# ChrisHird/ZLIB

Measured on AMD Instinct MI355X. Metric: GiB/s raw input compressed (deflate level 6), higher is better.
Workload: dtype u8

## Files before the change

### zlib_amd/csrc/zgpu_lz_parse.h

```cpp
#pragma once
#include "zgpu_common.h"

namespace zgpu {

#ifndef ZGPU_P2WIN
#define ZGPU_P2WIN 8192
#endif
constexpr uint32_t kP2Win = ZGPU_P2WIN, kP2Blk = kP2Win / 64;
constexpr uint32_t kP2Words = kChunkMax / 32, kP2Batch = 8, kP2Pair = 4, kP2Over = 8;
constexpr uint32_t kNone = 0xffffffffu;

struct ParseCtx {
    const uint2 *rec;
    uint32_t n, base, good, lazy, strategy;
    int slide_at;
    __device__ bool slid(uint32_t p) const { return (int)p >= slide_at; }
    __device__ uint32_t take(uint32_t p, uint32_t prev_len, uint2 r, uint32_t &dist) const
    {
        const uint32_t pick = (prev_len >= good && strategy != kRle) ? r.y : r.x;
        const uint32_t d = (pick >> 9) & 32767u;
        const bool nil = ((r.y >> 24) & 1u) && slid(p);
        const uint32_t len = nil ? 0u : (pick & 511u);
        const bool weak = len <= 5 && (strategy == kFiltered || (len == kMinMatch && d > kTooFar));
        const bool ok = prev_len < lazy && len > prev_len && !weak;
// ... 28 lines not shown
}

#if defined(ZGPU_P2_TIME) && !defined(ZGPU_PARSE_HEADER_ONLY)
__device__ unsigned long long p2_time[8];
extern "C" __attribute__((visibility("default"))) void zgpu_debug_p2_time(unsigned long long *out, int reset)
{
    unsigned long long z[8] = {};
    hipMemcpyFromSymbol(out, HIP_SYMBOL(p2_time), sizeof z);
    if (reset) hipMemcpyToSymbol(HIP_SYMBOL(p2_time), z, sizeof z);
}
#define P2_T(i) do { if (tid == 0) { const unsigned long long t_ = wall_clock64(); t_acc[i] += t_ - t_prev; t_prev = t_; } } while (0)
#define P2_T0() unsigned long long t_prev = wall_clock64(), t_acc[8] = {0, 0, 0, 0, 0, 0, 0, 0}
#define P2_TEND() do { if (tid == 0) for (int i_ = 0; i_ < 8; i_++) atomicAdd(&p2_time[i_], t_acc[i_]); } while (0)
#else
#define P2_T(i) do { } while (0)
#define P2_T0() do { } while (0)
#define P2_TEND() do { } while (0)
#endif

template <bool FUSED> __device__ inline uint32_t p2_ld(const uint32_t *p) { return FUSED ? __hip_atomic_load(p, __ATOMIC_RELAXED, __HIP_MEMORY_SCOPE_AGENT) : *p; }
constexpr uint32_t kP2OffJ = 0, kP2OffHAS = kP2Win * 2, kP2OffMARK = kP2OffHAS + kP2Words * 4, kP2OffCOV = kP2OffMARK + kP2Words * 4, kP2OffMAT = kP2OffCOV + kP2Words * 4,
                   kP2OffWbase = kP2OffMAT + kP2Words * 4, kP2OffVIS = kP2OffWbase + (kP2Words + 4) * 4, kP2OffEXITS = kP2OffVIS + kP2Win / 32 * 4, kP2OffWtot = kP2OffEXITS + 256,
                   kP2OffEntry = kP2OffWtot + 64, kP2LdsBytes = kP2OffEntry + 16;

}
```

### zlib_amd/csrc/zgpu_lz_parse.hip

```cpp
#include "zgpu_lz_parse.h"
#include "zgpu_engine.h"

namespace zgpu {

template <bool LITE, bool TILE>
__global__ void __launch_bounds__(1024, 8) parse2_kernel(ChunkGeom g, LevelCfg cfg, const uint2 *__restrict__ recs, const uint32_t *__restrict__ gmv_all,
                                                         const uint32_t *__restrict__ gsv_all, uint32_t *__restrict__ tokens, ChunkMeta *meta, TileGeom tg)
{
    constexpr uint32_t kP2Threads = 1024;
    constexpr bool FUSED = false;
    __shared__ __attribute__((aligned(16))) uint16_t J[kP2Win];
    __shared__ uint32_t HAS[kP2Words], MARK[kP2Words], COV[kP2Words], MAT[kP2Words];
    __shared__ uint32_t wbase[kP2Words + 1];
    __shared__ uint32_t VIS[kP2Win / 32], EXITS[64];
    __shared__ uint32_t wave_tot[kP2Threads / 64];
    __shared__ uint32_t sh_entry, sh_exit;
    const uint32_t c = blockIdx.x;
#include "zgpu_lz_parse_body.inc"
}

void launch_parse2(const ChunkGeom &g, LevelCfg cfg, const uint2 *recs, uint32_t *tokens, ChunkMeta *meta, hipStream_t st)
{
    hipLaunchKernelGGL((parse2_kernel<false, false>), dim3(g.nchunks), dim3(1024), 0, st, g, cfg, recs, nullptr, nullptr, tokens, meta, TileGeom{});
}

void launch_parse_tile(const ChunkGeom &g, LevelCfg cfg, const uint32_t *gm, const uint32_t *gs, uint32_t *tokens, ChunkMeta *meta, const TileGeom &tg, hipStream_t st)
{
    hipLaunchKernelGGL((parse2_kernel<true, true>), dim3(g.nchunks), dim3(1024), 0, st, g, cfg, nullptr, gm, gs, tokens, meta, tg);
}

}
```

### zlib_amd/csrc/zgpu_lz_parse_body.inc

```
{
    constexpr uint32_t kP2Own = kP2Win / kP2Threads;
    static_assert(kP2Own % kP2Batch == 0 && kP2Threads >= kP2Win / 32 && kP2Threads / 64 <= 16, "workgroup size");
    const uint32_t tid = threadIdx.x, lane = tid & 63, wave = tid >> 6;
    uint64_t lo; uint32_t n;
    chunk_span(g, c, lo, n);
    ParseCtx cx;
    cx.rec = LITE ? nullptr : recs + (size_t)c * kChunkMax;
    const uint32_t *gmv = LITE ? gmv_all + (size_t)c * kChunkMax : nullptr, *gsv = LITE ? gsv_all + (size_t)c * kP2Words : nullptr;
    cx.n = n; cx.base = chunk_base(g, c); cx.good = cfg.good; cx.lazy = cfg.lazy; cx.strategy = cfg.strategy;
    {
        const int room = (int)(2 * kWSize - cx.base), b0 = (int)n < room ? (int)n : room;
        const int a = b0 - (int)kMinLookahead + 1, b = (int)(kWSize + kMaxDist) - (int)cx.base;
        cx.slide_at = a > b ? a : b;
    }
    uint32_t *tok = tokens + (size_t)c * kChunkMax;
    const uint8_t *src = g.in + lo;
    const uint32_t nwords = (n + 31) >> 5;
    uint32_t t_h1 = n, t_e = 0;
    if (TILE) {
        uint64_t wb_; uint32_t nl_, h0_, ne_;
        tile_span(g, tg, c, wb_, nl_, h0_, t_h1, ne_);
        t_e = h0_ + tg.entry[g.chunk0 + c];
    }

    P2_T0();
    for (uint32_t i = tid; i < kP2Words; i += kP2Threads) { MARK[i] = 0; COV[i] = 0; MAT[i] = 0; if (LITE) HAS[i] = p2_ld<FUSED>(gsv + i); }
    if (!LITE) for (uint32_t p0 = 0; p0 < kChunkMax; p0 += kP2Threads * kP2Batch) {
        uint2 rv[kP2Batch];
#pragma unroll
        for (uint32_t u = 0; u < kP2Batch; u++) { const uint32_t p = p0 + u * kP2Threads + tid; rv[u] = p < n ? cx.rec[p] : make_uint2(0, 0); }
#pragma unroll
        for (uint32_t u = 0; u < kP2Batch; u++) {
            const uint32_t pw = p0 + u * kP2Threads, p = pw + tid;
            uint32_t d;
            const bool h = p < n && cx.take(p, kMinMatch - 1, rv[u], d) >= kMinMatch;
            const unsigned long long b = __builtin_amdgcn_ballot_w64(h);
            if (lane == 0) { HAS[(pw >> 5) + 2 * wave] = (uint32_t)b; HAS[(pw >> 5) + 2 * wave + 1] = (uint32_t)(b >> 32); }
        }
    }
    __syncthreads();
    if (tid == 0) {
        uint32_t x0 = (!TILE || t_e < t_h1) ? next_bit(HAS, t_e, nwords) : kNone;
        if (TILE && x0 != kNone && x0 >= t_h1) x0 = kNone;
        sh_entry = x0;
        if (TILE) sh_exit = t_e;
    }
    __syncthreads();
    P2_T(0);

    const uint32_t *TOK = COV;
    auto index_of = [&](uint32_t p) { return wbase[p >> 5] + (uint32_t)__builtin_popcount(TOK[p >> 5] & ~(~0u << (p & 31u))); };
    uint32_t tokbase = 0;
    uint32_t def_m = kNone, def_tok = 0;

    const uint32_t w_first = TILE ? t_e / kP2Win * kP2Win : 0u, w_lim = TILE ? (t_h1 + kTileSlack < n ? t_h1 + kTileSlack : n) : n;
    for (uint32_t w0 = w_first; w0 < w_lim; w0 += kP2Win) {
        const uint32_t wend = w0 + kP2Win;
        const uint32_t entry = sh_entry;
        uint32_t gm[kP2Own];
        uint32_t onp = 0;
#pragma unroll
        for (uint32_t i = 0; i < kP2Own; i++) gm[i] = 0;
        if (entry != kNone && entry < wend) {
            if (LITE) {
                uint32_t gv[kP2Own];
#pragma unroll
                for (uint32_t i = 0; i < kP2Own; i++) {
                    const uint32_t p = w0 + i * kP2Threads + tid;
#if defined(ZGPU_P2_EXP) && ZGPU_P2_EXP == 1
                    gv[i] = 0x00018001u;
#else
                    gv[i] = p < n ? p2_ld<FUSED>(gmv + p) : 0;
#endif
                }
#pragma unroll
                for (uint32_t i = 0; i < kP2Own; i++) {
                    const uint32_t p = w0 + i * kP2Threads + tid;
                    if (!(p < n && ((HAS[p >> 5] >> (p & 31u)) & 1u))) gv[i] = 0;
                }
#pragma unroll
                for (uint32_t i = 0; i < kP2Own; i++) {
                    const uint32_t xw = i * kP2Threads + tid, p = w0 + xw;
                    uint32_t succ = 0xffffu;
                    gm[i] = gv[i];
                    if (gv[i]) {
                        const uint32_t t = next_bit(HAS, p + (gv[i] >> 24) + ((gv[i] >> 15) & 511u), nwords);
                        if (t < wend) succ = t - w0;
// ... 125 lines not shown
                        if (x2 != kNone && x2 < be2) {
                            const uint32_t cw = (x2 - w0) >> 5;
                            if (lane < kP2Blk / 32) {
                                const uint32_t wd = blk * (kP2Blk / 32) + lane;
                                uint32_t v = VIS[wd];
                                if (wd < cw) v = 0; else if (wd == cw) v &= ~0u << (x2 & 31u);
                                if (v) atomicOr(&MARK[(w0 >> 5) + wd], v);
                            }
                            met_blk = blk;
                            x2 = EXITS[blk];
                        }
                        cur = (uint32_t)__builtin_amdgcn_readfirstlane(x2);
                        last = (uint32_t)__builtin_amdgcn_readfirstlane(last);
                        met_blk = (uint32_t)__builtin_amdgcn_readfirstlane(met_blk);
                    }
                    if (met_blk != kNone) {
                        uint32_t hi = 0;
                        for (uint32_t j = 0; j < kP2Blk / 32; j++) { const uint32_t v = VIS[met_blk * (kP2Blk / 32) + j]; if (v) hi = ((met_blk * (kP2Blk / 32) + j) << 5) + 32u - (uint32_t)__builtin_clz(v); }
                        last = w0 + hi - 1;
                    }
                }
                if (lane == 0) {
                    uint32_t m, L, D;
                    if (LITE) { const uint32_t gv = p2_ld<FUSED>(gmv + last); m = last + (gv >> 24); L = (gv >> 15) & 511u; D = gv & 32767u; }
                    else cx.game(last, cx.rec[last], cx.rec[last + 1], m, L, D);
                    sh_entry = next_bit(HAS, m + L, nwords);
                    if (TILE) sh_exit = m + L;
                }
            }
            __syncthreads();
            P2_T(2);
#pragma unroll
            for (uint32_t i = 0; i < kP2Own; i++) {
                const uint32_t p = w0 + i * kP2Threads + tid;
                const bool on_path = gm[i] != 0 && ((MARK[p >> 5] >> (p & 31u)) & 1u);
                onp |= on_path ? 1u << i : 0u;
                if (on_path) {
                    const uint32_t m = p + (gm[i] >> 24), L = (gm[i] >> 15) & 511u;
                    atomicOr(&MAT[m >> 5], 1u << (m & 31u));
                    const uint32_t a = m + 1, z = m + L;
                    for (uint32_t wd = a >> 5; wd <= (z - 1) >> 5; wd++) {
                        const uint32_t lo_b = wd == (a >> 5) ? (a & 31u) : 0u, hi_b = wd == ((z - 1) >> 5) ? ((z - 1) & 31u) : 31u;
                        atomicOr(&COV[wd], (~0u << lo_b) & (~0u >> (31u - hi_b)));
                    }
                }
            }
        }
        __syncthreads();
        P2_T(3);
        {
            const uint32_t wd = (w0 >> 5) + tid;
            uint32_t tw = 0;
            if (tid < kP2Win / 32 && wd < nwords) {
                tw = ~COV[wd];
                if (wd == nwords - 1 && (n & 31u)) tw &= ~0u >> (32u - (n & 31u));
                if (TILE) {
                    const uint32_t xl = wend > t_h1 ? (sh_exit > t_h1 ? sh_exit : t_h1) : wend, p0 = wd << 5;
// ... 10 lines not shown
            uint32_t b = tokbase + x - cnt, tot = 0;
            for (uint32_t w = 0; w < kP2Win / 32 / 64; w++) { const uint32_t t = wave_tot[w]; tot += t; if (w < wave) b += t; }
            if (tid < kP2Win / 32) { wbase[wd] = b; COV[wd] = tw; }
            tokbase += tot;
            __syncthreads();
        }
        P2_T(4);
        if (def_m != kNone) { tok[index_of(def_m)] = def_tok; def_m = kNone; }
#pragma unroll
        for (uint32_t ib = 0; ib < kP2Own; ib += kP2Batch) {
            uint32_t lit[kP2Batch];
            bool li[kP2Batch];
#pragma unroll
            for (uint32_t u = 0; u < kP2Batch; u++) {
                const uint32_t p = w0 + (ib + u) * kP2Threads + tid, bit = 1u << (p & 31u);
                li[u] = p < n && (TOK[p >> 5] & bit) && !(MAT[p >> 5] & bit);
                lit[u] = 0;
                if (p < n) lit[u] = src[p];
            }
#pragma unroll
            for (uint32_t u = 0; u < kP2Batch; u++) {
                const uint32_t p = w0 + (ib + u) * kP2Threads + tid;
                if (li[u]) tok[index_of(p)] = tok_lit(lit[u]);
                const uint32_t gv = ((onp >> (ib + u)) & 1u) ? gm[ib + u] : 0u;
                if (gv) {
                    const uint32_t m = p + (gv >> 24), t = tok_match(gv & 32767u, ((gv >> 15) & 511u) - kMinMatch);
                    if (m < wend) tok[index_of(m)] = t; else { def_m = m; def_tok = t; }
                }
            }
        }
        P2_T(5);
    }
    const uint32_t ntok = tokbase, nw_done = ((n + kP2Win - 1) / kP2Win) * (kP2Win / 32);
    __syncthreads();

    if (TILE) { if (tid == 0) { meta[c].ntok = ntok; meta[c].in_bytes = (sh_exit > t_h1 ? sh_exit : t_h1) - t_e; } }
    else if (tid == 0) {
        uint32_t nostore = 0, nblk = 0, block_start = 0;
        for (uint32_t b = 0;; b++) {
            const uint32_t e = (b + 1) * kBlockTokens - 1;
            if (e >= ntok) break;
            uint32_t lo_w = 0, hi_w = nw_done;
            while (hi_w - lo_w > 1) { const uint32_t mid = (lo_w + hi_w) >> 1; if (wbase[mid] <= e) lo_w = mid; else hi_w = mid; }
            uint32_t v = TOK[lo_w];
            for (uint32_t s2 = e - wbase[lo_w]; s2; s2--) v &= v - 1;
            const uint32_t pe = (lo_w << 5) + (uint32_t)__builtin_ctz(v);
            const bool is_mat = (MAT[pe >> 5] >> (pe & 31u)) & 1u;
            if (!is_mat && pe == n - 1) { nostore |= kFullFinalBlock; break; }
            uint32_t ns = pe + 1;
// ... 11 lines not shown
```

### zlib_amd/csrc/zgpu_lz_sorted.hip

```cpp
#include "zgpu_common.h"
#include "zgpu_engine.h"
#define ZGPU_PARSE_HEADER_ONLY
#include "zgpu_lz_parse.h"
#include <cstdlib>
#include "../../include/zamd_gpu.h"

#include <atomic>
static std::atomic<int> g_inject_sort_fault{0};
extern "C" __attribute__((visibility("default"))) void zgpu_debug_inject_sort_fault(void) { g_inject_sort_fault.store(1); }

namespace zgpu {

__device__ inline uint32_t lds_off(const void *p) { return (uint32_t)(uintptr_t)(const __attribute__((address_space(3))) void *)p; }
__device__ inline void lds_st32(uint32_t a, uint32_t v) { asm volatile("ds_write_b32 %0, %1" ::"v"(a), "v"(v) : "memory"); }
__device__ inline void lds_st16(uint32_t a, uint32_t v) { asm volatile("ds_write_b16 %0, %1" ::"v"(a), "v"(v) : "memory"); }
__device__ inline void lds_max32(uint32_t a, uint32_t v) { asm volatile("ds_max_u32 %0, %1" ::"v"(a), "v"(v) : "memory"); }
__device__ inline uint32_t lds_ld32(uint32_t a) { uint32_t v; asm volatile("ds_read_b32 %0, %1\n\ts_waitcnt lgkmcnt(0)" : "=v"(v) : "v"(a) : "memory"); return v; }
__device__ inline uint32_t lds_ld16(uint32_t a) { uint32_t v; asm volatile("ds_read_u16 %0, %1\n\ts_waitcnt lgkmcnt(0)" : "=v"(v) : "v"(a) : "memory"); return v; }

__device__ inline void lds_st8(uint32_t a, uint32_t v) { asm volatile("ds_write_b8 %0, %1" ::"v"(a), "v"(v) : "memory"); }
__device__ inline uint32_t lds_ld8(uint32_t a) { uint32_t v; asm volatile("ds_read_u8 %0, %1\n\ts_waitcnt lgkmcnt(0)" : "=v"(v) : "v"(a) : "memory"); return v; }

constexpr uint32_t kSuperS = 1024;

constexpr uint32_t kHeadWords = kChunkMax / 32;
constexpr uint32_t kHeadStride = kHeadWords + kChunkMax / 64 / 2;
constexpr uint32_t kGPad = 32, kGStride = kChunkMax + 2 * kGPad;

struct SortedWs {
    static constexpr size_t kHeaderBytes = 256, kSBytes = kSStride * 2, kRkBytes = kChunkMax * 2, kHeadBytes = kHeadStride * 4, kRecBytes = kChunkMax * 8, kIrBytes = kChunkMax * 4;
    static constexpr size_t kSlack = 1024;
    static_assert(kChunkMax * 4 + kChunkMax / 8 <= kRecBytes && kGStride <= kRecBytes, "gm + gs, and G, lie in the records' memory");
    static size_t bytes(size_t nchunks) { return kHeaderBytes + nchunks * (kSBytes + kRkBytes + kHeadBytes + kRecBytes + kIrBytes) + kSlack; }

    size_t nch;
    uint32_t *fault; uint16_t *S, *rk; uint32_t *heads; uint2 *recs; uint32_t *ir;
    SortedWs(void *workspace, size_t nchunks) : nch(nchunks)
    {
        uint8_t *p = static_cast<uint8_t *>(workspace);
        auto take = [&p](size_t n) { uint8_t *at = p; p += n; return at; };
        fault = reinterpret_cast<uint32_t *>(take(kHeaderBytes));
        S = reinterpret_cast<uint16_t *>(take((nch * kSBytes + 255) & ~(size_t)255));
        rk = reinterpret_cast<uint16_t *>(take(nch * kRkBytes));
        heads = reinterpret_cast<uint32_t *>(take(nch * kHeadBytes));
        recs = reinterpret_cast<uint2 *>(take(nch * kRecBytes));
        ir = reinterpret_cast<uint32_t *>(take(nch * kIrBytes));
    }
    uint32_t *gm() const { return reinterpret_cast<uint32_t *>(recs); }
    uint32_t *gs() const { return gm() + nch * kChunkMax; }
    uint8_t *G() const { return reinterpret_cast<uint8_t *>(recs); }
};

size_t lz_sorted_workspace_bytes(uint32_t batch) { return SortedWs::bytes(batch); }
uint32_t *lz_sorted_fault_word(void *workspace) { return SortedWs(workspace, 0).fault; }

__device__ inline uint32_t heads_below(unsigned long long x, uint32_t tid, uint32_t *wave_scratch)
{
    const uint32_t lane = tid & 63, wave = tid >> 6;
    const uint32_t v = x ? 64u * tid + 64u - (uint32_t)__builtin_clzll(x) : 0;
    uint32_t inc = v;
#pragma unroll
    for (int d = 1; d < 64; d <<= 1) { const uint32_t y = __shfl_up(inc, d); if ((int)lane >= d && y > inc) inc = y; }
    if (lane == 63) wave_scratch[wave] = inc;
    __syncthreads();
    uint32_t ex = __shfl_up(inc, 1);
    if (lane == 0) ex = 0;
    for (uint32_t w = 0; w < wave; w++) { const uint32_t y = wave_scratch[w]; if (y > ex) ex = y; }
    const uint32_t dist = 64u * tid - (ex - 1);
    return ex && dist < 65535u ? dist : 65535u;
}

__global__ void __launch_bounds__(1024) heads_below_kernel(uint32_t *__restrict__ heads_all)
// ... 531 lines not shown
            }
            if (p + base == kWSize + kMaxDist && avail != 0 && (uint32_t)sp[-1] + base == kWSize) flags = 1;
            rec[p] = make_uint2(full | ((uint32_t)d8[p] << 24), snap | (flags << 24));
        }
        blk = blk_nx;
    }
}

#ifndef ZGPU_WTRIG
#define ZGPU_WTRIG 48
#endif
#ifndef ZGPU_WBLK
#define ZGPU_WBLK 64
#endif
#ifndef ZGPU_WNEU_SHIFT
#define ZGPU_WNEU_SHIFT 0
#endif
#ifndef ZGPU_WFOLD_AT
#define ZGPU_WFOLD_AT 64
#endif
constexpr uint32_t kWFoldAt = ZGPU_WFOLD_AT;
constexpr uint32_t kWThreads = 512, kWWaves = kWThreads / 64, kWBlk = ZGPU_WBLK, kWTrig = ZGPU_WTRIG, kWNeuShift = ZGPU_WNEU_SHIFT;
constexpr uint32_t kWNeuBytes = (kChunkMax >> kWNeuShift) / 8;
constexpr uint32_t kWLds = kM3DataLds + 16 + kWNeuBytes + kWWaves * kM3WaveLds;
static_assert(2 * kWLds <= 160 * 1024, "two walker workgroups per CU");
enum : uint32_t { W_NEED = 0, W_LIMBO = 1, W_READY = 2, W_SEARCH = 3, W_DONE = 4 };
#ifdef ZGPU_WALK_STATS
__device__ unsigned long long walk_stats[8];
extern "C" __attribute__((visibility("default"))) void zgpu_debug_walk_stats(unsigned long long *out, int reset)
{
    unsigned long long z[8] = {};
    hipMemcpyFromSymbol(out, HIP_SYMBOL(walk_stats), sizeof z);
    if (reset) hipMemcpyToSymbol(HIP_SYMBOL(walk_stats), z, sizeof z);
}
#define W_STAT(i, v) do { const unsigned long long v_ = (unsigned long long)(v); if (lane == 0) atomicAdd(&walk_stats[i], v_); } while (0)
#else
#define W_STAT(i, v) do { } while (0)
#endif
#ifdef ZGPU_WALK_TIME
__device__ unsigned long long walk_time[8];
extern "C" __attribute__((visibility("default"))) void zgpu_debug_walk_time(unsigned long long *out, int reset)
{
    unsigned long long z[8] = {};
    hipMemcpyFromSymbol(out, HIP_SYMBOL(walk_time), sizeof z);
    if (reset) hipMemcpyToSymbol(HIP_SYMBOL(walk_time), z, sizeof z);
}
#define W_T0() unsigned long long wt_prev = __builtin_readcyclecounter(), wt_fold = 0, wt_lds = 0, wt_take = 0, wt_acc[8] = {0, 0, 0, 0, 0, 0, 0, 0}
#define W_T(i) do { const unsigned long long t_ = __builtin_readcyclecounter(); wt_acc[i] += t_ - wt_prev - ((i) == 1 ? wt_fold + wt_lds + wt_take : 0); \
                    if ((i) == 1) { wt_acc[2] += wt_fold; wt_acc[3] += wt_lds; wt_acc[7] += wt_take; } wt_fold = wt_lds = wt_take = 0; wt_prev = t_; } while (0)
#define W_TF(stmt) do { const unsigned long long f0_ = __builtin_readcyclecounter(); stmt; wt_fold += __builtin_readcyclecounter() - f0_; } while (0)
#define W_TL(stmt) do { const unsigned long long f0_ = __builtin_readcyclecounter(); stmt; wt_lds += __builtin_readcyclecounter() - f0_; } while (0)
#define W_TK(stmt) do { const unsigned long long f0_ = __builtin_readcyclecounter(); asm volatile("s_waitcnt vmcnt(0)" ::: "memory"); stmt; wt_take += __builtin_readcyclecounter() - f0_; } while (0)
#define W_TEND() do { if (lane == 0) for (int i_ = 0; i_ < 8; i_++) atomicAdd(&walk_time[i_], wt_acc[i_]); } while (0)
#else
#define W_T0() do { } while (0)
#define W_T(i) do { } while (0)
#define W_TF(stmt) stmt
#define W_TL(stmt) stmt
// ... 70 lines not shown
                N[rank_of(p)] = (uint16_t)v;
            }
        }
    }
    __syncthreads();
    for (;;) {
        bool more = false;
        for (uint32_t i = tid; i < nn; i += T) {
            const uint32_t v = N[i];
            if (!(v & kExit)) { const uint32_t w = N[v]; N[i] = (uint16_t)w; more = more || !(w & kExit); }
        }
        if (!__syncthreads_or(more)) break;
    }
    for (uint32_t k = tid; k < kTileExitStride; k += T) {
        uint32_t v = 0;
        if (k < nent) {
            const uint32_t e = h0 + k, t = e < h1 ? next_bit(HAS, e, kWords) : kNone;
            v = (t == kNone || t >= h1) ? (e > h1 ? e - h1 : 0u) : ((uint32_t)N[rank_of(t)] & 0x7fffu);
        }
        exits[k] = (uint16_t)v;
    }
}

static_assert(kP2LdsBytes <= kM3DataLds, "the parse works in the memory of the chunk bytes");
template <int MODE>
__global__ void __launch_bounds__(kWThreads, kWThreads / 128) walk_kernel(ChunkGeom g, LevelCfg cfg, const uint16_t *__restrict__ S_all, const uint32_t *__restrict__ ir_all,
                                                            uint32_t *__restrict__ gm_all, uint32_t *__restrict__ gs_all, uint32_t *__restrict__ tokens, ChunkMeta *meta, TileGeom tg)
{
    static_assert(MODE == 1 || MODE == 2, "a chunk or a tile");
    constexpr bool FUSE = MODE == 1, TILE = MODE == 2;
    extern __shared__ __attribute__((aligned(16))) uint32_t lds[];
    uint32_t *d32 = lds;
    uint32_t *ctrl = lds + kM3DataLds / 4;
    uint32_t *NEU = ctrl + 4;
    const uint8_t *d8 = reinterpret_cast<const uint8_t *>(d32);
    const uint32_t c = blockIdx.x, tid = threadIdx.x, lane = tid & 63, wave = tid >> 6;
    const uint32_t ring = (uint32_t)__builtin_amdgcn_readfirstlane(lds_off(lds) + kM3DataLds + 16 + kWNeuBytes + wave * kM3WaveLds), slot = ring + kRing * 4, pw = slot + 64 * 4;
    uint64_t lo; uint32_t n;
    chunk_span(g, c, lo, n);
    const uint8_t *src = g.in + lo;
    const uint16_t *S = S_all + (size_t)c * kSStride + kSPad;
    const uint32_t *ir = ir_all + (size_t)c * kChunkMax;
    uint32_t *gm = gm_all + (size_t)c * kChunkMax, *gs = gs_all + (size_t)c * (kChunkMax / 32);
    uint32_t th0 = 0, th1 = n, tnent = 0, tnent_all = 0, nil_local = ~0u;
    uint32_t base = chunk_base(g, c);
    if (TILE) {
        uint64_t wb; uint32_t nl;
        tile_span(g, tg, c, wb, nl, th0, th1, tnent);
        tnent_all = tnent;
        if (tnent > th1 - th0) tnent = th1 - th0;
        base = (tg.abs0_nil && tg.abs0 + wb == 0) ? 0u : 1u;
        if (tg.nil_pos >= wb && tg.nil_pos - wb < kChunkMax) nil_local = (uint32_t)(tg.nil_pos - wb);
    }
    const uint32_t npos = n >= 3 ? n - 2 : 0;
    stage_chunk<kWThreads>(src, n, d32, tid);
    for (uint32_t i = tid; i < kChunkMax / 32; i += kWThreads) { if (i < kWNeuBytes / 4) NEU[i] = 0; gs[i] = 0; }
    if (tid < 8) d32[(kChunkMax + 64) / 4 + tid] = 0xffffffffu;
    if (tid == 0) ctrl[0] = 0;
    __syncthreads();
    int slide_at;
    {
        const int room = (int)(2 * kWSize - base), b0 = (int)n < room ? (int)n : room;
        const int a = b0 - (int)kMinLookahead + 1, b = (int)(kWSize + kMaxDist) - (int)base;
        slide_at = a > b ? a : b;
    }
    const uint32_t chainF = cfg.chain, chainQ = cfg.chain >> 2, dbase = lds_off(d32), nblk = TILE ? tnent + (th1 - th0 - tnent + kWBlk - 1) / kWBlk : (n + kWBlk - 1) / kWBlk;
    const uint32_t wlim = TILE ? th1 : n;
    const bool vexact = (chainF & 7u) != 0 || (chainQ & 7u) != 0 || cfg.strategy == kRle;
    const uint32_t lanebits = lane << 16, dummy = ring + (kRing - 1) * 4;
    uint32_t st = W_NEED, x = 0, handL = kMinMatch - 1, handM = 0, handD = 0, gstart = 0;
    uint32_t irx = 0, irn = 0, irE = 0, irl = 0;
    bool haveE = false;
    uint32_t rem = 0, best = kMinMatch - 1, key_seen = 0, sentinel = 0, scan2 = 0, boff = dbase + 1;
    int gi = -(int)kSPad;
    uint32_t firstb = 0;
    uint4 G0 = make_uint4(0, 0, 0, 0), G1 = G0, G2 = G0, G3 = G0, F0 = G0, F1 = G0, F2 = G0, F3 = G0;
    uint32_t left = 0;
    bool cont = false;
    unsigned long long amask = 0, jmask = 0;
    uint32_t tail = 0;

// ... 36 lines not shown
        const bool fin = st == W_SEARCH && !(((amask | jmask) >> lane) & 1ull) && !cont;
        W_STAT(2, 1); W_STAT(3, __popcll(__builtin_amdgcn_ballot_w64(fin || st == W_LIMBO || st == W_NEED)));
        if (st == W_LIMBO) { irx = irl; st = W_READY; }
        uint32_t y = 0, irY = 0;
        bool toN = false, haveIr = false;
        if (fin) {
            uint32_t len = kMinMatch - 1, dist = 0;
            if (key_seen != sentinel) {
                const bool nz = key_seen >> 31;
                len = nz ? key_seen & 0x1ffu : key_seen >> 16;
                dist = x - (nz ? (key_seen >> 9) & 0xffffu : key_seen & 0xffffu);
            }
            if (len <= 5 && (cfg.strategy == kFiltered || (len == kMinMatch && dist > kTooFar))) len = kMinMatch - 1;
            bool emit = false;
            if (len > handL) {
                if (handL < kMinMatch) gstart = x;
                handL = len; handD = dist; handM = x;
                if (len < cfg.lazy && x + 1 < npos) { x = x + 1; irx = irn; st = W_READY; }
                else emit = true;
                haveE = false;
            } else if (handL >= kMinMatch) emit = true;
            else { y = x + 1; irY = irn; toN = haveIr = true; }
            if (emit) {
                gm[gstart] = ((handM - gstart) << 24) | (handL << 15) | handD;
                atomicOr(&gs[gstart >> 5], 1u << (gstart & 31u));
                y = handM + handL; irY = irE; haveIr = haveE; toN = true;
                handL = kMinMatch - 1;
            }
        }
        if (toN) {
            st = W_NEED;
            if (y < wlim) {
                const uint32_t yc = y >> kWNeuShift, bit = 1u << (yc & 31u);
                const bool meet = (y & ((1u << kWNeuShift) - 1u)) == 0;
                if (!meet || !(atomicOr(&NEU[yc >> 5], bit) & bit)) {
                    x = y;
                    if (haveIr) { irx = irY; st = W_READY; }
                    else { irl = y < npos ? ir[y] : 0; st = W_LIMBO; W_STAT(7, 1); }
                }
            }
        }
        W_T(5);
        {
            const unsigned long long nm = __builtin_amdgcn_ballot_w64(st == W_NEED);
            if (nm) {
                const int first = __builtin_ctzll(nm);
                uint32_t b0 = 0;
                if ((int)lane == first) b0 = atomicAdd(&ctrl[0], (uint32_t)__popcll(nm));
// ... 124 lines not shown
            }
            G0 = G1; G1 = G2; G2 = G3;
            left = left ? left - 1 : 0;
            if (first && jmask) {
                W_TK(if ((jmask >> lane) & 1ull) { G0 = F0; G1 = F1; G2 = F2; G3 = F3; left = 4; });
            }
            rem = sel_mask(amask0, rem > 8 ? rem - 8 : 0, rem);
            {
                const unsigned long long cm = amask & mask_eq_u32(left, 0u);
                cont = cont || ((cm >> lane) & 1ull);
                amask &= ~cm;
            }
            amask |= jmask; jmask = 0;
            if (amask == 0 || (uint32_t)__popcll(smask & ~amask) + idle >= kWTrig) break;
        }
        W_T(1);
    }
    if (TILE) {
        __syncthreads();
        tile_exits<kWThreads>(reinterpret_cast<uint8_t *>(lds), gm, gs, th0, th1, tnent_all, tg.exits + (size_t)c * kTileExitStride, tid);
    }
    if (FUSE) {
        __syncthreads();
        constexpr uint32_t kP2Threads = kWThreads;
        constexpr bool LITE = true, FUSED = true, TILE = false;
        const uint2 *recs = nullptr;
        const uint32_t *gmv_all = gm_all, *gsv_all = gs_all;
        uint8_t *pl = reinterpret_cast<uint8_t *>(lds);
        uint16_t *const J = reinterpret_cast<uint16_t *>(pl + kP2OffJ);
        uint32_t *const HAS = reinterpret_cast<uint32_t *>(pl + kP2OffHAS), *const MARK = reinterpret_cast<uint32_t *>(pl + kP2OffMARK), *const COV = reinterpret_cast<uint32_t *>(pl + kP2OffCOV),
                 *const MAT = reinterpret_cast<uint32_t *>(pl + kP2OffMAT), *const wbase = reinterpret_cast<uint32_t *>(pl + kP2OffWbase), *const VIS = reinterpret_cast<uint32_t *>(pl + kP2OffVIS),
                 *const EXITS = reinterpret_cast<uint32_t *>(pl + kP2OffEXITS), *const wave_tot = reinterpret_cast<uint32_t *>(pl + kP2OffWtot);
        uint32_t &sh_entry = *reinterpret_cast<uint32_t *>(pl + kP2OffEntry), &sh_exit = *reinterpret_cast<uint32_t *>(pl + kP2OffEntry + 4);
#include "zgpu_lz_parse_body.inc"
    }
}

struct __attribute__((packed, aligned(1))) U128b { uint4 v; };
enum : uint32_t { F_IR = 0, F_GROUP, F_CAND, F_EXT, F_DONE };

__device__ inline uint32_t first_diff16(uint4 a, uint4 b)
{
    const uint64_t x0 = (((uint64_t)(a.y ^ b.y)) << 32) | (a.x ^ b.x), x1 = (((uint64_t)(a.w ^ b.w)) << 32) | (a.z ^ b.z);
    return x0 ? (uint32_t)__builtin_ctzll(x0) >> 3 : x1 ? 8 + ((uint32_t)__builtin_ctzll(x1) >> 3) : 16u;
}

__device__ __noinline__ uint4 tail16(const uint8_t *in, uint32_t o, uint64_t safe_end)
{
    uint32_t v[4] = {0, 0, 0, 0};
    for (uint32_t k = 0; k < 16 && (uint64_t)o + k < safe_end; k++) v[k >> 2] |= (uint32_t)in[o + k] << (8 * (k & 3));
    return make_uint4(v[0], v[1], v[2], v[3]);
}

__global__ void __launch_bounds__(64) fast_kernel(ChunkGeom g, LevelCfg cfg, const uint16_t *__restrict__ S_all, const uint32_t *__restrict__ ir_all, uint8_t *G_all,
                                                   uint32_t *__restrict__ tokens, ChunkMeta *meta, uint32_t lanes)
{
// ... 153 lines not shown

static bool launch_sort(const ChunkGeom &g, const SortedWs &ws, ChunkMeta *meta, hipStream_t st, zgpu_engine *prof, int exact_sort)
{
    static int sort_env = -1;
    if (sort_env < 0) { const char *e = getenv("ZGPU_SORT"); sort_env = e ? atoi(e) : 4; }
    const bool exact = exact_sort || sort_env == 1;
    hipEvent_t ev{};
    prof_span_begin(prof, st, &ev);
    if (exact) {
        hipLaunchKernelGGL(sort_kernel, dim3(g.nchunks), dim3(kSortThreads), 0, st, g, ws.S, ws.rk, ws.heads, ws.ir);
        hipLaunchKernelGGL(heads_below_kernel, dim3(g.nchunks), dim3(1024), 0, st, ws.heads);
    } else {
        hipLaunchKernelGGL(sort4_kernel, dim3(g.nchunks), dim3(kS4Threads), 0, st, g, ws.S, ws.heads, ws.fault, ws.ir, meta);
        if (g_inject_sort_fault.exchange(0)) hipMemsetAsync(ws.fault, 1, 4, st);
    }
    prof_span_end(prof, st, ZGPU_STAGE_CHAIN, ev);
    return !exact;
}

template <int MODE> static void launch_walk(const ChunkGeom &g, LevelCfg cfg, const SortedWs &ws, uint32_t *tokens, ChunkMeta *meta, const TileGeom &tg, hipStream_t st)
{
    static bool opt_in = false;
    if (!opt_in) { hipFuncSetAttribute(reinterpret_cast<const void *>(walk_kernel<MODE>), hipFuncAttributeMaxDynamicSharedMemorySize, (int)kWLds); opt_in = true; }
    hipLaunchKernelGGL(walk_kernel<MODE>, dim3(g.nchunks), dim3(kWThreads), kWLds, st, g, cfg, ws.S, ws.ir, ws.gm(), ws.gs(), tokens, meta, tg);
}

bool launch_lz_sorted(const ChunkGeom &g, LevelCfg cfg, void *workspace, uint32_t *tokens, ChunkMeta *meta, hipStream_t st, zgpu_engine *prof, int exact_sort, int impl)
{
    const SortedWs ws(workspace, g.nchunks);
    const bool adler_done = launch_sort(g, ws, meta, st, prof, exact_sort);
    hipEvent_t ev{};
    prof_span_begin(prof, st, &ev);
    if (impl == ZGPU_LZ_FASTWIN) launch_lz_fastwin(g, cfg, ws.S, ws.ir, tokens, meta, st);
    else if (impl == ZGPU_LZ_FAST) {
        hipMemsetAsync(ws.G(), 0, ws.nch * kGStride, st);
        static int forced = -1;
        if (forced < 0) { const char *v = getenv("ZGPU_FAST_LANES"); forced = v ? atoi(v) : 0; if (forced < 0 || forced > 64) forced = 0; }
        uint32_t lanes = (uint32_t)forced;
        if (!lanes) { lanes = 1; while (lanes < 64 && (uint64_t)lanes * 4096 < g.nchunks) lanes <<= 1; }
        hipLaunchKernelGGL(fast_kernel, dim3((g.nchunks + lanes - 1) / lanes), dim3(64), 0, st, g, cfg, ws.S, ws.ir, ws.G(), tokens, meta, lanes);
    } else if (impl == ZGPU_LZ_WALK) launch_walk<1>(g, cfg, ws, tokens, meta, TileGeom{}, st);
    else {
        static bool opt_in3 = false;
        if (!opt_in3) { hipFuncSetAttribute(reinterpret_cast<const void *>(match3_kernel), hipFuncAttributeMaxDynamicSharedMemorySize, (int)kM3Lds); opt_in3 = true; }
        hipLaunchKernelGGL(match3_kernel, dim3(g.nchunks), dim3(kM2Threads), kM3Lds, st, g, cfg, ws.S, ws.heads, ws.recs);
        prof_span_end(prof, st, ZGPU_STAGE_MATCH, ev);
        prof_span_begin(prof, st, &ev);
// ... 39 lines not shown
```

### zlib_amd/gpu.py

```python
import ctypes as C
import os

_HERE = os.path.dirname(os.path.abspath(__file__))
_lib = None

F_FINAL, F_ZLIB_WRAP, F_POS0, F_POS0_ALL, F_GZIP_WRAP, F_CRC32, F_CONTINUOUS, F_BGZF_WRAP = 1, 2, 4, 8, 16, 32, 64, 128
BGZF_BLOCK = 65280
CONT_MORE, CONT_FLUSH, CONT_FINISH = 0, 1, 2
WHOLE_STREAM = 0xFFFFFFFF
LZ_AUTO, LZ_SERIAL, LZ_PARALLEL, LZ_SORTED, LZ_WALK, LZ_FAST, LZ_FASTWIN = 0, 1, 2, 3, 4, 5, 6
CHECK_ADLER32, CHECK_CRC32 = 1, 2
WRAP_RAW, WRAP_ZLIB, WRAP_GZIP, WRAP_AUTO = 0, 1, 2, 3
_WRAPS = {"raw": WRAP_RAW, "zlib": WRAP_ZLIB, "gzip": WRAP_GZIP, "auto": WRAP_AUTO}
BUF_ERROR = -5
STAGES = ["chain", "match", "parse", "lz_serial", "huffman", "stitch", "inflate"]
CHUNK = 65536


class EngineError(RuntimeError):
    def __init__(self, code, msg):
        super().__init__("zgpu error %d: %s" % (code, msg))
        self.code = code


# ... 39 lines not shown
    if _lib is not None:
        return _lib
    try:
        import torch
    except ImportError:
        pass
    path = library_path()
    if not os.path.exists(path):
        raise ImportError("%s is missing: build it with `make -C zlib_amd/csrc` (or __graft_entry__.build())" % path)
    L = C.CDLL(path)
    vp, u64, u32 = C.c_void_p, C.c_uint64, C.c_uint32
    L.zgpu_device_count.restype = C.c_int
    L.zgpu_engine_create.argtypes = [C.c_int, C.POINTER(vp)]
    L.zgpu_engine_destroy.argtypes = [vp]
    L.zgpu_engine_destroy.restype = None
    L.zgpu_engine_error.argtypes = [vp]
    L.zgpu_engine_error.restype = C.c_char_p
    L.zgpu_version.restype = C.c_char_p
    L.zgpu_deflate_bound.argtypes = [u64, u32]
    L.zgpu_deflate_bound.restype = u64
    L.zgpu_deflate_bound_geometry.argtypes = [u64, u32, C.c_int, C.c_int]
    L.zgpu_deflate_bound_geometry.restype = u64
    L.zgpu_deflate_set_geometry.argtypes = [vp, C.c_int, C.c_int]
    L.zgpu_deflate_device.argtypes = [vp, vp, u64, C.POINTER(_Params), vp, u64, vp, C.POINTER(DeflateResult), vp]
    L.zgpu_deflate_host.argtypes = [vp, vp, u64, C.POINTER(_Params), vp, u64, vp, C.POINTER(DeflateResult)]
    L.zgpu_deflate_cont_bound.argtypes = [u64]
    L.zgpu_deflate_cont_bound.restype = u64
    L.zgpu_deflate_cont_host.argtypes = [vp, vp, u64, vp, u64, u64, C.POINTER(_Params), C.c_int, C.POINTER(ContState), vp, vp, vp, u32, vp, u64, C.POINTER(DeflateResult)]
    L.zgpu_deflate_segments_host.argtypes = [vp, vp, vp, u64, C.POINTER(_Params), vp, u64, vp, C.POINTER(DeflateResult)]
    L.zgpu_deflate_segments_device.argtypes = [vp, vp, u64, vp, u64, C.POINTER(_Params), vp, u64, vp, C.POINTER(DeflateResult), vp]
    L.zgpu_deflate_segments_items_host.argtypes = [vp, vp, vp, u64, C.POINTER(_Params), vp, u64, vp, C.POINTER(DeflateResult), vp]
    L.zgpu_deflate_segments_items_device.argtypes = [vp, vp, u64, vp, u64, C.POINTER(_Params), vp, u64, vp, C.POINTER(DeflateResult), vp, vp]
    L.zgpu_checksum_batch_host.argtypes = [vp, vp, u64, vp, u64, u32, vp]
    L.zgpu_checksum_batch_device.argtypes = [vp, vp, u64, vp, u64, u32, vp, vp]
    L.zgpu_inflate_device.argtypes = [vp, vp, u64, vp, u64, u32, vp, u64, C.POINTER(InflateResult), vp]
    L.zgpu_inflate_host.argtypes = [vp, vp, u64, vp, u64, u32, vp, u64, C.POINTER(InflateResult)]
    L.zgpu_deflate_segments_bound.argtypes = [u64, u64, u32]
    L.zgpu_deflate_segments_bound.restype = u64
    L.zgpu_inflate_batch_device.argtypes = [vp, vp, u64, vp, u64, C.c_int, u32, vp, u64, vp, vp, C.POINTER(u64), vp]
    L.zgpu_inflate_batch_host.argtypes = [vp, vp, u64, vp, u64, C.c_int, u32, vp, u64, vp, vp, C.POINTER(u64)]
    L.zgpu_inflate_batch_sizes_device.argtypes = [vp, vp, u64, vp, u64, C.c_int, vp, C.POINTER(u64), vp]
    L.zgpu_inflate_batch_sizes_host.argtypes = [vp, vp, u64, vp, u64, C.c_int, vp, C.POINTER(u64)]
    L.zgpu_inflate_batch_packed_device.argtypes = [vp, vp, u64, vp, u64, C.c_int, u32, u32, vp, u64, vp, vp, C.POINTER(u64), C.POINTER(u64), vp]
    L.zgpu_inflate_batch_packed_host.argtypes = [vp, vp, u64, vp, u64, C.c_int, u32, u32, vp, u64, vp, vp, C.POINTER(u64), C.POINTER(u64)]
    L.zgpu_bgzf_bound.argtypes = [u64, u32]
    L.zgpu_bgzf_bound.restype = u64
# ... 107 lines not shown
        import numpy as np
        cs = ContState(0, 0, 0, 0, 0, 0, 2, 1, 8)
        return cs, (np.zeros(16384, dtype=np.uint32), np.zeros(1040, dtype=np.uint32))

    def deflate_cont_host(self, buf, check_from, level, mode, cs, carry, strategy=0, flags=0, excl=(), split=None):
        import numpy as np
        arr = np.frombuffer(bytes(buf) + b"\0", dtype=np.uint8)
        n = int(arr.size) - 1
        split = 0 if split is None else min(max(split, 0), n)
        cap = self.L.zgpu_deflate_cont_bound(n) + 64
        out = np.empty(cap, dtype=np.uint8)
        p = _Params(level, 0, flags, LZ_AUTO, strategy, 0)
        res = DeflateResult()
        ex = np.ascontiguousarray(list(excl) + [0], dtype=np.uint64)
        self._check(self.L.zgpu_deflate_cont_host(self.h, arr.ctypes.data, split, arr.ctypes.data + split, n - split, check_from, C.byref(p), mode, C.byref(cs), carry[0].ctypes.data,
                                                  carry[1].ctypes.data, ex.ctypes.data, len(excl), out.ctypes.data, cap, C.byref(res)))
        self.last = res
        return out[: res.out_bytes].tobytes()

    def set_geometry(self, window_bits=15, mem_level=8):
        self._check(self.L.zgpu_deflate_set_geometry(self.h, window_bits, mem_level))
        self.geometry = (window_bits, mem_level)

    def deflate_segments_host(self, buffers, level, flags=0, lz_impl=LZ_AUTO, want_items=False):
        import numpy as np
        sizes = [len(b) for b in buffers]
        offs = np.zeros(len(buffers) + 1, dtype=np.uint64)
        offs[1:] = np.cumsum(sizes)
        blob = np.frombuffer(b"".join(buffers) + b"\0", dtype=np.uint8)
        cap = int(offs[-1]) + 40 * len(buffers) + 64
        if getattr(self, "geometry", (15, 8)) != (15, 8):
            cap = int(offs[-1]) + len(buffers) * (12288 + 5 * 520)
        out = np.empty(cap, dtype=np.uint8)
        ooffs = np.zeros(len(buffers) + 1, dtype=np.uint64)
        p = _Params(level, 0, flags, lz_impl)
        res = DeflateResult()
        if want_items:
            cap += 26 * len(buffers)
            out = np.empty(cap, dtype=np.uint8)
            items = (DeflateItem * max(len(buffers), 1))()
            self._check(self.L.zgpu_deflate_segments_items_host(self.h, blob.ctypes.data, offs.ctypes.data, len(buffers), C.byref(p),
                                                                out.ctypes.data, cap, ooffs.ctypes.data, C.byref(res), items))
        else:
            self._check(self.L.zgpu_deflate_segments_host(self.h, blob.ctypes.data, offs.ctypes.data, len(buffers), C.byref(p),
                                                          out.ctypes.data, cap, ooffs.ctypes.data, C.byref(res)))
        self.last = res
        raw = out[: res.out_bytes].tobytes()
        segs = [raw[int(ooffs[i]): int(ooffs[i + 1])] for i in range(len(buffers))]
        if want_items:
            return segs, [(it.out_lo, it.out_bytes, it.in_bytes, it.data_type, it.adler32, it.crc32) for it in items[: len(buffers)]]
        return segs

    def checksum_batch_host(self, data, offsets, checks=CHECK_ADLER32 | CHECK_CRC32, items=None):
        import numpy as np
        arr = data if hasattr(data, "ctypes") else np.frombuffer(bytes(data) + b"\0", dtype=np.uint8)[:-1]
        offs = np.ascontiguousarray(offsets, dtype=np.uint64)
        n = len(offs) - 1
        given = items is not None
# ... 325 lines not shown
```

Before: 27.38.

## Have fused walker log per-window game starts compactly for the parse stage

In the fused walk+parse kernel, walkers now append each emitted game (record and 16-bit start position) to a per-window log using an LDS counter, instead of scattering records into a chunk-sized gm array and setting bits in a global gs bitmap. The parse body rebuilds HAS from the logs and loads only logged games per window, computing jump targets and game ends from them. The aim is to cut global atomics and sparse scans over mostly empty positions, at the cost of LDS atomics for log slots, an extra END array in LDS, and a separate token emission loop. Python bindings for set_tuning and a strategy parameter are also added.

```diff
diff --git a/zlib_amd/csrc/zgpu_lz_parse.h b/zlib_amd/csrc/zgpu_lz_parse.h
--- a/zlib_amd/csrc/zgpu_lz_parse.h
+++ b/zlib_amd/csrc/zgpu_lz_parse.h
@@ -74,5 +74,7 @@
 constexpr uint32_t kP2OffJ = 0, kP2OffHAS = kP2Win * 2, kP2OffMARK = kP2OffHAS + kP2Words * 4, kP2OffCOV = kP2OffMARK + kP2Words * 4, kP2OffMAT = kP2OffCOV + kP2Words * 4,
                    kP2OffWbase = kP2OffMAT + kP2Words * 4, kP2OffVIS = kP2OffWbase + (kP2Words + 4) * 4, kP2OffEXITS = kP2OffVIS + kP2Win / 32 * 4, kP2OffWtot = kP2OffEXITS + 256,
                    kP2OffEntry = kP2OffWtot + 64, kP2LdsBytes = kP2OffEntry + 16;
+constexpr uint32_t kP2Wins = kChunkMax / kP2Win, kP2OffEND = kP2LdsBytes, kP2LogLdsBytes = kP2OffEND + kP2Win * 2;
+static_assert(kChunkMax % kP2Win == 0 && kP2Win - 1 + 255 + 258 <= 0xffffu, "whole windows; a game's end fits END");
 
 }
diff --git a/zlib_amd/csrc/zgpu_lz_parse.hip b/zlib_amd/csrc/zgpu_lz_parse.hip
--- a/zlib_amd/csrc/zgpu_lz_parse.hip
+++ b/zlib_amd/csrc/zgpu_lz_parse.hip
@@ -8,7 +8,8 @@
                                                          const uint32_t *__restrict__ gsv_all, uint32_t *__restrict__ tokens, ChunkMeta *meta, TileGeom tg)
 {
     constexpr uint32_t kP2Threads = 1024;
-    constexpr bool FUSED = false;
+    constexpr bool FUSED = false, LOG = false;
+    const uint16_t *const lpos = nullptr; const uint32_t *const lrec = nullptr, *const lcnt = nullptr; uint16_t *const END = nullptr;
     __shared__ __attribute__((aligned(16))) uint16_t J[kP2Win];
     __shared__ uint32_t HAS[kP2Words], MARK[kP2Words], COV[kP2Words], MAT[kP2Words];
     __shared__ uint32_t wbase[kP2Words + 1];
diff --git a/zlib_amd/csrc/zgpu_lz_parse_body.inc b/zlib_amd/csrc/zgpu_lz_parse_body.inc
--- a/zlib_amd/csrc/zgpu_lz_parse_body.inc
+++ b/zlib_amd/csrc/zgpu_lz_parse_body.inc
@@ -23,8 +23,26 @@
         t_e = h0_ + tg.entry[g.chunk0 + c];
     }
 
+    static_assert(!LOG || (LITE && !TILE), "the logs are what a chunk's walkers leave");
     P2_T0();
-    for (uint32_t i = tid; i < kP2Words; i += kP2Threads) { MARK[i] = 0; COV[i] = 0; MAT[i] = 0; if (LITE) HAS[i] = p2_ld<FUSED>(gsv + i); }
+    for (uint32_t i = tid; i < kP2Words; i += kP2Threads) { MARK[i] = 0; COV[i] = 0; MAT[i] = 0; if (LOG) HAS[i] = 0; else if (LITE) HAS[i] = p2_ld<FUSED>(gsv + i); }
+    const uint32_t *lpos2 = reinterpret_cast<const uint32_t *>(lpos);
+    if (LOG) {
+        constexpr uint32_t kRounds = kP2Win / 2 / kP2Threads;
+        __syncthreads();
+        for (uint32_t w = 0; w < kP2Wins; w++) {
+            const uint32_t cw = (uint32_t)__builtin_amdgcn_readfirstlane((int)lcnt[w]);
+            uint32_t pv[kRounds];
+#pragma unroll
+            for (uint32_t r = 0; r < kRounds; r++) { pv[r] = 0; if (r * kP2Threads * 2 < cw) pv[r] = p2_ld<FUSED>(lpos2 + w * (kP2Win / 2) + r * kP2Threads + tid); }
+#pragma unroll
+            for (uint32_t r = 0; r < kRounds; r++) {
+                const uint32_t e = (r * kP2Threads + tid) * 2, p0 = pv[r] & 0xffffu, p1 = pv[r] >> 16;
+                if (e < cw) atomicOr(&HAS[p0 >> 5], 1u << (p0 & 31u));
+                if (e + 1 < cw) atomicOr(&HAS[p1 >> 5], 1u << (p1 & 31u));
+            }
+        }
+    }
     if (!LITE) for (uint32_t p0 = 0; p0 < kChunkMax; p0 += kP2Threads * kP2Batch) {
         uint2 rv[kP2Batch];
 #pragma unroll
@@ -58,11 +76,33 @@
         const uint32_t wend = w0 + kP2Win;
         const uint32_t entry = sh_entry;
         uint32_t gm[kP2Own];
+        uint32_t gp[kP2Own];
         uint32_t onp = 0;
 #pragma unroll
-        for (uint32_t i = 0; i < kP2Own; i++) gm[i] = 0;
+        for (uint32_t i = 0; i < kP2Own; i++) { gm[i] = 0; gp[i] = 0; }
+        auto pos_of = [&](uint32_t i) { return LOG ? gp[i] : w0 + i * kP2Threads + tid; };
         if (entry != kNone && entry < wend) {
-            if (LITE) {
+            if (LOG) {
+                const uint32_t cw = (uint32_t)__builtin_amdgcn_readfirstlane((int)lcnt[w0 / kP2Win]);
+                const uint32_t *lp2 = lpos2 + w0 / 2, *lr = lrec + w0;
+                uint32_t gv[kP2Own], gq[kP2Own];
+#pragma unroll
+                for (uint32_t i = 0; i < kP2Own; i++) {
+                    gv[i] = 0; gq[i] = 0;
+                    if (i * kP2Threads < cw) { const uint32_t e = i * kP2Threads + tid; gq[i] = p2_ld<FUSED>(lp2 + (e >> 1)); gv[i] = p2_ld<FUSED>(lr + e); }
+                }
+#pragma unroll
+                for (uint32_t i = 0; i < kP2Own; i++) {
+                    const bool v = i * kP2Threads + tid < cw;
+                    const uint32_t p = (gq[i] >> ((tid & 1u) << 4)) & 0xffffu;
+                    gm[i] = v ? gv[i] : 0u; gp[i] = v ? p : 0u;
+                    if (v) {
+                        const uint32_t end = p + (gv[i] >> 24) + ((gv[i] >> 15) & 511u), t = next_bit(HAS, end, nwords);
+                        J[p - w0] = (uint16_t)(t < wend ? t - w0 : 0xffffu);
+                        END[p - w0] = (uint16_t)(end - w0);
+                    }
+                }
+            } else if (LITE) {
                 uint32_t gv[kP2Own];
 #pragma unroll
                 for (uint32_t i = 0; i < kP2Own; i++) {
@@ -234,7 +274,8 @@
                 }
                 if (lane == 0) {
                     uint32_t m, L, D;
-                    if (LITE) { const uint32_t gv = p2_ld<FUSED>(gmv + last); m = last + (gv >> 24); L = (gv >> 15) & 511u; D = gv & 32767u; }
+                    if (LOG) { m = w0 + END[last - w0]; L = 0; }
+                    else if (LITE) { const uint32_t gv = p2_ld<FUSED>(gmv + last); m = last + (gv >> 24); L = (gv >> 15) & 511u; D = gv & 32767u; }
                     else cx.game(last, cx.rec[last], cx.rec[last + 1], m, L, D);
                     sh_entry = next_bit(HAS, m + L, nwords);
                     if (TILE) sh_exit = m + L;
@@ -244,7 +285,7 @@
             P2_T(2);
 #pragma unroll
             for (uint32_t i = 0; i < kP2Own; i++) {
-                const uint32_t p = w0 + i * kP2Threads + tid;
+                const uint32_t p = pos_of(i);
                 const bool on_path = gm[i] != 0 && ((MARK[p >> 5] >> (p & 31u)) & 1u);
                 onp |= on_path ? 1u << i : 0u;
                 if (on_path) {
@@ -301,9 +342,19 @@
             for (uint32_t u = 0; u < kP2Batch; u++) {
                 const uint32_t p = w0 + (ib + u) * kP2Threads + tid;
                 if (li[u]) tok[index_of(p)] = tok_lit(lit[u]);
-                const uint32_t gv = ((onp >> (ib + u)) & 1u) ? gm[ib + u] : 0u;
+                const uint32_t gv = (!LOG && ((onp >> (ib + u)) & 1u)) ? gm[ib + u] : 0u;
                 if (gv) {
                     const uint32_t m = p + (gv >> 24), t = tok_match(gv & 32767u, ((gv >> 15) & 511u) - kMinMatch);
+                    if (m < wend) tok[index_of(m)] = t; else { def_m = m; def_tok = t; }
+                }
+            }
+        }
+        if (LOG) {
+#pragma unroll
+            for (uint32_t i = 0; i < kP2Own; i++) {
+                const uint32_t gv = ((onp >> i) & 1u) ? gm[i] : 0u;
+                if (gv) {
+                    const uint32_t m = gp[i] + (gv >> 24), t = tok_match(gv & 32767u, ((gv >> 15) & 511u) - kMinMatch);
                     if (m < wend) tok[index_of(m)] = t; else { def_m = m; def_tok = t; }
                 }
             }
diff --git a/zlib_amd/csrc/zgpu_lz_sorted.hip b/zlib_amd/csrc/zgpu_lz_sorted.hip
--- a/zlib_amd/csrc/zgpu_lz_sorted.hip
+++ b/zlib_amd/csrc/zgpu_lz_sorted.hip
@@ -31,6 +31,7 @@
     static constexpr size_t kHeaderBytes = 256, kSBytes = kSStride * 2, kRkBytes = kChunkMax * 2, kHeadBytes = kHeadStride * 4, kRecBytes = kChunkMax * 8, kIrBytes = kChunkMax * 4;
     static constexpr size_t kSlack = 1024;
     static_assert(kChunkMax * 4 + kChunkMax / 8 <= kRecBytes && kGStride <= kRecBytes, "gm + gs, and G, lie in the records' memory");
+    static_assert(kChunkMax * (4 + 2) <= kRecBytes, "and so do the logs: the workspace, and with it the batch a device holds, is what it was");
     static size_t bytes(size_t nchunks) { return kHeaderBytes + nchunks * (kSBytes + kRkBytes + kHeadBytes + kRecBytes + kIrBytes) + kSlack; }
 
     size_t nch;
@@ -48,6 +49,8 @@
     }
     uint32_t *gm() const { return reinterpret_cast<uint32_t *>(recs); }
     uint32_t *gs() const { return gm() + nch * kChunkMax; }
+    uint32_t *lrec() const { return reinterpret_cast<uint32_t *>(recs); }
+    uint16_t *lpos() const { return reinterpret_cast<uint16_t *>(lrec() + nch * kChunkMax); }
     uint8_t *G() const { return reinterpret_cast<uint8_t *>(recs); }
 };
 
@@ -625,7 +628,8 @@
 constexpr uint32_t kWFoldAt = ZGPU_WFOLD_AT;
 constexpr uint32_t kWThreads = 512, kWWaves = kWThreads / 64, kWBlk = ZGPU_WBLK, kWTrig = ZGPU_WTRIG, kWNeuShift = ZGPU_WNEU_SHIFT;
 constexpr uint32_t kWNeuBytes = (kChunkMax >> kWNeuShift) / 8;
-constexpr uint32_t kWLds = kM3DataLds + 16 + kWNeuBytes + kWWaves * kM3WaveLds;
+constexpr uint32_t kWOffLcnt = kM3DataLds + 16 + kWNeuBytes + kWWaves * kM3WaveLds;
+constexpr uint32_t kWLds = kWOffLcnt + kP2Wins * 4;
 static_assert(2 * kWLds <= 160 * 1024, "two walker workgroups per CU");
 enum : uint32_t { W_NEED = 0, W_LIMBO = 1, W_READY = 2, W_SEARCH = 3, W_DONE = 4 };
 #ifdef ZGPU_WALK_STATS
@@ -637,6 +641,13 @@
     if (reset) hipMemcpyToSymbol(HIP_SYMBOL(walk_stats), z, sizeof z);
 }
 #define W_STAT(i, v) do { const unsigned long long v_ = (unsigned long long)(v); if (lane == 0) atomicAdd(&walk_stats[i], v_); } while (0)
+__device__ unsigned long long walk_log_stats[2];
+extern "C" __attribute__((visibility("default"))) void zgpu_debug_walk_log_stats(unsigned long long *out, int reset)
+{
+    unsigned long long z[2] = {};
+    hipMemcpyFromSymbol(out, HIP_SYMBOL(walk_log_stats), sizeof z);
+    if (reset) hipMemcpyToSymbol(HIP_SYMBOL(walk_log_stats), z, sizeof z);
+}
 #else
 #define W_STAT(i, v) do { } while (0)
 #endif
@@ -753,17 +764,19 @@
     }
 }
 
-static_assert(kP2LdsBytes <= kM3DataLds, "the parse works in the memory of the chunk bytes");
+static_assert(kP2LogLdsBytes <= kWOffLcnt, "the parse works in the memory of the chunk bytes, the neutral bitmap and the rings");
 template <int MODE>
 __global__ void __launch_bounds__(kWThreads, kWThreads / 128) walk_kernel(ChunkGeom g, LevelCfg cfg, const uint16_t *__restrict__ S_all, const uint32_t *__restrict__ ir_all,
                                                             uint32_t *__restrict__ gm_all, uint32_t *__restrict__ gs_all, uint32_t *__restrict__ tokens, ChunkMeta *meta, TileGeom tg)
 {
     static_assert(MODE == 1 || MODE == 2, "a chunk or a tile");
     constexpr bool FUSE = MODE == 1, TILE = MODE == 2;
+    static_assert(!FUSE || kWNeuShift == 0, "a log holds kP2Win games: a position must start one game at most, so every neutral position is claimed");
     extern __shared__ __attribute__((aligned(16))) uint32_t lds[];
     uint32_t *d32 = lds;
     uint32_t *ctrl = lds + kM3DataLds / 4;
     uint32_t *NEU = ctrl + 4;
+    uint32_t *lcnt = lds + kWOffLcnt / 4;
     const uint8_t *d8 = reinterpret_cast<const uint8_t *>(d32);
     const uint32_t c = blockIdx.x, tid = threadIdx.x, lane = tid & 63, wave = tid >> 6;
     const uint32_t ring = (uint32_t)__builtin_amdgcn_readfirstlane(lds_off(lds) + kM3DataLds + 16 + kWNeuBytes + wave * kM3WaveLds), slot = ring + kRing * 4, pw = slot + 64 * 4;
@@ -773,6 +786,7 @@
     const uint16_t *S = S_all + (size_t)c * kSStride + kSPad;
     const uint32_t *ir = ir_all + (size_t)c * kChunkMax;
     uint32_t *gm = gm_all + (size_t)c * kChunkMax, *gs = gs_all + (size_t)c * (kChunkMax / 32);
+    uint32_t *lrec = gm; uint16_t *lpos = reinterpret_cast<uint16_t *>(gs_all) + (size_t)c * kChunkMax;
     uint32_t th0 = 0, th1 = n, tnent = 0, tnent_all = 0, nil_local = ~0u;
     uint32_t base = chunk_base(g, c);
     if (TILE) {
@@ -785,9 +799,10 @@
     }
     const uint32_t npos = n >= 3 ? n - 2 : 0;
     stage_chunk<kWThreads>(src, n, d32, tid);
-    for (uint32_t i = tid; i < kChunkMax / 32; i += kWThreads) { if (i < kWNeuBytes / 4) NEU[i] = 0; gs[i] = 0; }
+    for (uint32_t i = tid; i < kChunkMax / 32; i += kWThreads) { if (i < kWNeuBytes / 4) NEU[i] = 0; if (!FUSE) gs[i] = 0; }
     if (tid < 8) d32[(kChunkMax + 64) / 4 + tid] = 0xffffffffu;
     if (tid == 0) ctrl[0] = 0;
+    if (FUSE && tid < kP2Wins) lcnt[tid] = 0;
     __syncthreads();
     int slide_at;
     {
@@ -870,8 +885,14 @@
             } else if (handL >= kMinMatch) emit = true;
             else { y = x + 1; irY = irn; toN = haveIr = true; }
             if (emit) {
-                gm[gstart] = ((handM - gstart) << 24) | (handL << 15) | handD;
-                atomicOr(&gs[gstart >> 5], 1u << (gstart & 31u));
+                const uint32_t rec = ((handM - gstart) << 24) | (handL << 15) | handD;
+                if (FUSE) {
+                    const uint32_t w = gstart / kP2Win, at = w * kP2Win + atomicAdd(&lcnt[w], 1u);
+                    lrec[at] = rec; lpos[at] = (uint16_t)gstart;
+                } else {
+                    gm[gstart] = rec;
+                    atomicOr(&gs[gstart >> 5], 1u << (gstart & 31u));
+                }
                 y = handM + handL; irY = irE; haveIr = haveE; toN = true;
                 handL = kMinMatch - 1;
             }
@@ -1042,16 +1063,20 @@
     }
     if (FUSE) {
         __syncthreads();
+#ifdef ZGPU_WALK_STATS
+        if (tid < kP2Wins) { atomicAdd(&walk_log_stats[0], (unsigned long long)lcnt[tid]); atomicMax(&walk_log_stats[1], (unsigned long long)lcnt[tid]); }
+#endif
         constexpr uint32_t kP2Threads = kWThreads;
-        constexpr bool LITE = true, FUSED = true, TILE = false;
+        constexpr bool LITE = true, FUSED = true, TILE = false, LOG = true;
         const uint2 *recs = nullptr;
-        const uint32_t *gmv_all = gm_all, *gsv_all = gs_all;
+        const uint32_t *gmv_all = nullptr, *gsv_all = nullptr;
         uint8_t *pl = reinterpret_cast<uint8_t *>(lds);
         uint16_t *const J = reinterpret_cast<uint16_t *>(pl + kP2OffJ);
         uint32_t *const HAS = reinterpret_cast<uint32_t *>(pl + kP2OffHAS), *const MARK = reinterpret_cast<uint32_t *>(pl + kP2OffMARK), *const COV = reinterpret_cast<uint32_t *>(pl + kP2OffCOV),
                  *const MAT = reinterpret_cast<uint32_t *>(pl + kP2OffMAT), *const wbase = reinterpret_cast<uint32_t *>(pl + kP2OffWbase), *const VIS = reinterpret_cast<uint32_t *>(pl + kP2OffVIS),
                  *const EXITS = reinterpret_cast<uint32_t *>(pl + kP2OffEXITS), *const wave_tot = reinterpret_cast<uint32_t *>(pl + kP2OffWtot);
         uint32_t &sh_entry = *reinterpret_cast<uint32_t *>(pl + kP2OffEntry), &sh_exit = *reinterpret_cast<uint32_t *>(pl + kP2OffEntry + 4);
+        uint16_t *const END = reinterpret_cast<uint16_t *>(pl + kP2OffEND);
 #include "zgpu_lz_parse_body.inc"
     }
 }
@@ -1251,7 +1276,8 @@
 {
     static bool opt_in = false;
     if (!opt_in) { hipFuncSetAttribute(reinterpret_cast<const void *>(walk_kernel<MODE>), hipFuncAttributeMaxDynamicSharedMemorySize, (int)kWLds); opt_in = true; }
-    hipLaunchKernelGGL(walk_kernel<MODE>, dim3(g.nchunks), dim3(kWThreads), kWLds, st, g, cfg, ws.S, ws.ir, ws.gm(), ws.gs(), tokens, meta, tg);
+    uint32_t *games = MODE == 1 ? ws.lrec() : ws.gm(), *starts = MODE == 1 ? reinterpret_cast<uint32_t *>(ws.lpos()) : ws.gs();
+    hipLaunchKernelGGL(walk_kernel<MODE>, dim3(g.nchunks), dim3(kWThreads), kWLds, st, g, cfg, ws.S, ws.ir, games, starts, tokens, meta, tg);
 }
 
 bool launch_lz_sorted(const ChunkGeom &g, LevelCfg cfg, void *workspace, uint32_t *tokens, ChunkMeta *meta, hipStream_t st, zgpu_engine *prof, int exact_sort, int impl)
diff --git a/zlib_amd/gpu.py b/zlib_amd/gpu.py
--- a/zlib_amd/gpu.py
+++ b/zlib_amd/gpu.py
@@ -85,6 +85,7 @@
     L.zgpu_deflate_bound_geometry.argtypes = [u64, u32, C.c_int, C.c_int]
     L.zgpu_deflate_bound_geometry.restype = u64
     L.zgpu_deflate_set_geometry.argtypes = [vp, C.c_int, C.c_int]
+    L.zgpu_deflate_set_tuning.argtypes = [vp, C.c_int, u32, u32, u32, u32]
     L.zgpu_deflate_device.argtypes = [vp, vp, u64, C.POINTER(_Params), vp, u64, vp, C.POINTER(DeflateResult), vp]
     L.zgpu_deflate_host.argtypes = [vp, vp, u64, C.POINTER(_Params), vp, u64, vp, C.POINTER(DeflateResult)]
     L.zgpu_deflate_cont_bound.argtypes = [u64]
@@ -238,7 +239,11 @@
         self._check(self.L.zgpu_deflate_set_geometry(self.h, window_bits, mem_level))
         self.geometry = (window_bits, mem_level)
 
-    def deflate_segments_host(self, buffers, level, flags=0, lz_impl=LZ_AUTO, want_items=False):
+    def set_tuning(self, tune=None):
+        g, l, n, c = tune if tune else (0, 0, 0, 0)
+        self._check(self.L.zgpu_deflate_set_tuning(self.h, 1 if tune else 0, g, l, n, c))
+
+    def deflate_segments_host(self, buffers, level, flags=0, lz_impl=LZ_AUTO, want_items=False, strategy=0):
         import numpy as np
         sizes = [len(b) for b in buffers]
         offs = np.zeros(len(buffers) + 1, dtype=np.uint64)
@@ -249,7 +254,7 @@
             cap = int(offs[-1]) + len(buffers) * (12288 + 5 * 520)
         out = np.empty(cap, dtype=np.uint8)
         ooffs = np.zeros(len(buffers) + 1, dtype=np.uint64)
-        p = _Params(level, 0, flags, lz_impl)
+        p = _Params(level, 0, flags, lz_impl, strategy, 0)
         res = DeflateResult()
         if want_items:
             cap += 26 * len(buffers)
```

After: 28.51, median of 6. +4.1%, better.
